# Dane-ME/keypoint-detection

Measured on AMD Instinct MI355X. Metric: images/sec @ 256x192 COCO-17 (MultiPersonKeypointModel.forward, given boxes), higher is better.
Workload: dtype fp32; 1 GPU; C2: batch 64/GPU, 256x192x3, 1 box/img, heatmap head + soft-argmax decode; model=MultiPersonKeypointModel (MobileNetV3-Small+FPN, HeatmapHead), global_batch=64, height=256, width=192, persons=1, precision=split, parallelism=dp1, streams_per_gpu=1, gather=False, gather_pipelined=False

## Files before the change

### keypoint-detection_amd/csrc/head_kernels.hip

```cpp
#include <algorithm>

#include "kpd_common.h"
#include "kpd_kernels.h"

namespace {
constexpr int HM = 56;
static_assert(HM % 4 == 0, "hm_spool / hm_sapply take 4 pixels per load instruction");
constexpr int HMP = HM * HM;
constexpr int NK = 17;
constexpr int TOPK = 64;
constexpr int FC = 128;

__device__ __forceinline__ void slotmap_image(const float* __restrict__ boxes, int b, int P, int32_t* __restrict__ slot);
__global__ __launch_bounds__(256) void topk_kernel(const float* __restrict__ stats, int tiles, int HW,
                                                   const float* __restrict__ w0, const float* __restrict__ b0,
                                                   const float* __restrict__ w2, const float* __restrict__ b2,
                                                   int32_t* __restrict__ topk, float* __restrict__ scores_out,
                                                   const float* __restrict__ boxes, int P, int32_t* __restrict__ slot,
                                                   float* __restrict__ imax, float* __restrict__ sc_zero, int sc_n) {
  extern __shared__ __attribute__((aligned(16))) float tsm[];
  float* sw0 = tsm;
  float* sw2 = sw0 + 8 * FC;
  __shared__ float avg[FC], mx[FC], h[16], sc[FC];
  const int n = blockIdx.x, tid = threadIdx.x, c = tid;
// ... 550 lines not shown
                                                       const float* __restrict__ smap, const float* __restrict__ saw,
                                                       const float* __restrict__ sab, void* __restrict__ xs,
                                                       int out_bf16, const float* __restrict__ hsc, int use_sp,
                                                       float* __restrict__ sw_out) {
  constexpr int NI = HM / 4;
  __shared__ float w[98];
  __shared__ float2 srow[7][HM + 6];
  __shared__ float ssw[HM];
  const int y = blockIdx.x, r = blockIdx.y, x = threadIdx.x, pp = x >> 4, c = x & 15;
  const float* sm = smap + (size_t)r * HMP * 2;
  const float4* src = reinterpret_cast<const float4*>(roi + ((size_t)r * HM + y) * HM * TOPK);
  float4 v[NI];
  {
#pragma unroll
    for (int i = 0; i < NI; ++i) v[i] = src[(4 * i + pp) * (TOPK / 4) + c];
    float2 sv[7];
#pragma unroll
    for (int ky = 0; ky < 7; ++ky) {
      const int iy = y + ky - 3;
      sv[ky] = (x < HM && iy >= 0 && iy < HM) ? *reinterpret_cast<const float2*>(sm + (iy * HM + x) * 2)
                                                : make_float2(0.f, 0.f);
    }
    const float w0v = saw[x], w1v = x + 64 < 98 ? saw[x + 64] : 0.f;
#pragma unroll
    for (int ky = 0; ky < 7; ++ky) {
      if (x < HM) srow[ky][x + 3] = sv[ky];
      if (x < 3) { srow[ky][x] = make_float2(0.f, 0.f); srow[ky][HM + 3 + x] = make_float2(0.f, 0.f); }
    }
    w[x] = w0v;
    if (x + 64 < 98) w[x + 64] = w1v;
  }
  __syncthreads();
  if (x < HM) {
    float a = 0.f;
#pragma unroll
    for (int ky = 0; ky < 7; ++ky) {
      const int iy = y + ky - 3;
      if (iy < 0 || iy >= HM) continue;
#pragma unroll
      for (int kx = 0; kx < 7; ++kx) {
        const int ix = x + kx - 3;
        if (ix < 0 || ix >= HM) continue;
        const float2 sv2 = srow[ky][x + kx];
        a = fmaf(w[ky * 7 + kx], sv2.x, a);
        a = fmaf(w[49 + ky * 7 + kx], sv2.y, a);
      }
    }
    ssw[x] = use_sp ? kpd_sigmoid(a + sab[0]) : 1.f;
    if (sw_out) sw_out[((size_t)r * HM + y) * HM + x] = ssw[x];
  }
  const float4 cq = reinterpret_cast<const float4*>(cw + (size_t)r * TOPK)[c];
  const float ssc = out_bf16 == 3 ? ldexpf(1.f, split_exp_of(hsc[(size_t)r * 4])) : 1.f;
  __syncthreads();
#pragma unroll
  for (int i = 0; i < NI; ++i) {
    const int px = 4 * i + pp;
    const float sw = ssw[px];
    const float4 o = make_float4((v[i].x * cq.x) * sw, (v[i].y * cq.y) * sw, (v[i].z * cq.z) * sw, (v[i].w * cq.w) * sw);
    if (out_bf16 == 3) {
      const size_t opix = hm_pos(r, y, px);
      const float ov[4] = {o.x * ssc, o.y * ssc, o.z * ssc, o.w * ssc};
      f16x4 hi, lo;
#pragma unroll
      for (int e = 0; e < 4; ++e) {
        hi[e] = (_Float16)ov[e];
        lo[e] = (_Float16)(ov[e] - (float)hi[e]);
      }
      _Float16* ob = reinterpret_cast<_Float16*>(xs) + opix * 2 * TOPK + (c >> 3) * 64 + (c & 7) * 4;
      *reinterpret_cast<f16x4*>(ob) = hi;
      *reinterpret_cast<f16x4*>(ob + 32) = lo;
    } else if (out_bf16) {
      const size_t opix = out_bf16 == 2 ? hm_pos(r, y, px)
                                        : ((size_t)r * HM + y) * HM + px;
      bf16x4 ob;
      ob[0] = (__bf16)o.x; ob[1] = (__bf16)o.y; ob[2] = (__bf16)o.z; ob[3] = (__bf16)o.w;
      *reinterpret_cast<bf16x4*>(reinterpret_cast<__bf16*>(xs) + opix * TOPK + 4 * c) = ob;
    } else {
      reinterpret_cast<float4*>(reinterpret_cast<float*>(xs) + (((size_t)r * HM + y) * HM + px) * TOPK)[c] = o;
    }
  }
}

constexpr int kAttBR = 8;
__global__ __launch_bounds__(512) void hm_attn_kernel(const float* __restrict__ roi, const float* __restrict__ cw,
                                                      const float* __restrict__ saw, const float* __restrict__ sab,
                                                      void* __restrict__ xs, int out_bf16, const float* __restrict__ hsc,
                                                      int use_sp, float* __restrict__ sw_out) {
  constexpr int NI = HM / 4, BR = kAttBR, PR = BR + 6;
  __shared__ float w[98];
  __shared__ float2 pool[PR][HM + 6];
  __shared__ float ssw[BR][HM];
  const int nb = HM / BR;
  const int nblk = gridDim.x, L = blockIdx.x;
  const int qx = nblk / 8, rx = nblk % 8, x8 = L % 8, k8 = L / 8;
  const int g = (x8 < rx ? x8 * (qx + 1) : rx * (qx + 1) + (x8 - rx) * qx) + k8;
  const int r = g / nb, y0 = (g - r * nb) * BR;
  const int tid = threadIdx.x, lane = tid & 63, wave = tid >> 6, pp = lane >> 4, c = lane & 15;
  const float4 cq = reinterpret_cast<const float4*>(cw + (size_t)r * TOPK)[c];
  if (tid < 98) w[tid] = saw[tid];
  for (int i = tid; i < PR * 6; i += 512) {
    const int rr = i / 6, cc = i - rr * 6;
    pool[rr][cc < 3 ? cc : HM + cc] = make_float2(0.f, 0.f);
  }
  for (int pr = wave; pr < PR; pr += 8) {
    const int y = y0 - 3 + pr;
    if (y < 0 || y >= HM) {
      if (lane < HM) pool[pr][lane + 3] = make_float2(0.f, 0.f);
      continue;
    }
    const float4* src = reinterpret_cast<const float4*>(roi + ((size_t)r * HM + y) * HM * TOPK);
    float4 v[NI];
#pragma unroll
    for (int i = 0; i < NI; ++i) v[i] = src[(4 * i + pp) * (TOPK / 4) + c];
#pragma unroll
    for (int i = 0; i < NI; ++i) {
      const float a = v[i].x * cq.x, b = v[i].y * cq.y, cc = v[i].z * cq.z, d = v[i].w * cq.w;
      float sm = (a + b) + (cc + d), m = fmaxf(fmaxf(a, b), fmaxf(cc, d));
      sm += dpp_f<0xB1>(sm); m = fmaxf(m, dpp_f<0xB1>(m));
      sm += dpp_f<0x4E>(sm); m = fmaxf(m, dpp_f<0x4E>(m));
      sm += dpp_f<0x124>(sm); m = fmaxf(m, dpp_f<0x124>(m));
      sm += dpp_f<0x128>(sm); m = fmaxf(m, dpp_f<0x128>(m));
      if (c == 0) pool[pr][4 * i + pp + 3] = make_float2(sm / (float)TOPK, m);
    }
  }
  __syncthreads();
  if (tid < BR * HM) {
    const int j = tid / HM, x = tid - j * HM, y = y0 + j;
    float a = 0.f;
#pragma unroll
    for (int ky = 0; ky < 7; ++ky) {
      const int iy = y + ky - 3;
      if (iy < 0 || iy >= HM) continue;
#pragma unroll
      for (int kx = 0; kx < 7; ++kx) {
        const int ix = x + kx - 3;
        if (ix < 0 || ix >= HM) continue;
        const float2 sv2 = pool[j + ky][x + kx];
        a = fmaf(w[ky * 7 + kx], sv2.x, a);
        a = fmaf(w[49 + ky * 7 + kx], sv2.y, a);
      }
    }
    ssw[j][x] = use_sp ? kpd_sigmoid(a + sab[0]) : 1.f;
    if (sw_out) sw_out[((size_t)r * HM + y) * HM + x] = ssw[j][x];
  }
  const float ssc = out_bf16 == 3 ? ldexpf(1.f, split_exp_of(hsc[(size_t)r * 4])) : 1.f;
  __syncthreads();
  {
    const int j = wave, y = y0 + j;
    const float4* src = reinterpret_cast<const float4*>(roi + ((size_t)r * HM + y) * HM * TOPK);
    float4 v[NI];
#pragma unroll
    for (int i = 0; i < NI; ++i) v[i] = src[(4 * i + pp) * (TOPK / 4) + c];
#pragma unroll
    for (int i = 0; i < NI; ++i) {
      const int px = 4 * i + pp;
      const float sw = ssw[j][px];
      const float4 o = make_float4((v[i].x * cq.x) * sw, (v[i].y * cq.y) * sw, (v[i].z * cq.z) * sw, (v[i].w * cq.w) * sw);
      if (out_bf16 == 3) {
        const size_t opix = hm_pos(r, y, px);
        const float ov[4] = {o.x * ssc, o.y * ssc, o.z * ssc, o.w * ssc};
        f16x4 hi, lo;
#pragma unroll
        for (int e = 0; e < 4; ++e) {
          hi[e] = (_Float16)ov[e];
          lo[e] = (_Float16)(ov[e] - (float)hi[e]);
        }
        _Float16* ob = reinterpret_cast<_Float16*>(xs) + opix * 2 * TOPK + (c >> 3) * 64 + (c & 7) * 4;
        *reinterpret_cast<f16x4*>(ob) = hi;
        *reinterpret_cast<f16x4*>(ob + 32) = lo;
      } else if (out_bf16) {
        const size_t opix = out_bf16 == 2 ? hm_pos(r, y, px)
                                          : ((size_t)r * HM + y) * HM + px;
        bf16x4 ob;
        ob[0] = (__bf16)o.x; ob[1] = (__bf16)o.y; ob[2] = (__bf16)o.z; ob[3] = (__bf16)o.w;
        *reinterpret_cast<bf16x4*>(reinterpret_cast<__bf16*>(xs) + opix * TOPK + 4 * c) = ob;
      } else {
        reinterpret_cast<float4*>(reinterpret_cast<float*>(xs) + (((size_t)r * HM + y) * HM + px) * TOPK)[c] = o;
      }
    }
  }
}

__global__ __launch_bounds__(64) void hm_final_kernel(const float* __restrict__ h3, const float* __restrict__ w,
                                                      const float* __restrict__ b, const int32_t* __restrict__ slot,
                                                      int P, float* __restrict__ heat_out) {
  __shared__ float sw[NK * TOPK];
  __shared__ float sb[NK];
  const int y = blockIdx.x, r = blockIdx.y, x = threadIdx.x;
  const int sl = slot[r];
  if (sl < 0) {
    if (x < HM) {
      float* dst = heat_out + ((size_t)((r / P) * P + slot_pos(sl)) * NK) * HMP + y * HM + x;
      for (int k = 0; k < NK; ++k) dst[(size_t)k * HMP] = 0.f;
    }
    return;
  }
  for (int i = x; i < NK * TOPK; i += 64) sw[i] = w[i];
  if (x < NK) sb[x] = b[x];
  __syncthreads();
  if (x >= HM) return;
  const int bimg = r / P;
  const size_t pix = ((size_t)r * HM + y) * HM + x;
  float v[TOPK];
  const float4* src = reinterpret_cast<const float4*>(h3 + pix * TOPK);
#pragma unroll
  for (int q = 0; q < TOPK / 4; ++q) {
    const float4 u = src[q];
    v[4 * q] = u.x; v[4 * q + 1] = u.y; v[4 * q + 2] = u.z; v[4 * q + 3] = u.w;
  }
  float* dst = heat_out + ((size_t)(bimg * P + sl) * NK) * HMP + y * HM + x;
  for (int k = 0; k < NK; ++k) {
    float a = 0.f;
#pragma unroll
    for (int c = 0; c < TOPK; ++c) a = fmaf(sw[k * TOPK + c], v[c], a);
    dst[(size_t)k * HMP] = kpd_sigmoid(a + sb[k]);
  }
}

__global__ __launch_bounds__(64) void decode_kernel(const float* __restrict__ heat_out,
                                                    const float* __restrict__ boxes,
                                                    const int32_t* __restrict__ slot, int P,
                                                    float* __restrict__ kpts_out, float* __restrict__ vis_out) {
  const int r = blockIdx.x, k = blockIdx.y, lane = threadIdx.x;
  const int sl = slot[r];
  const int bimg = r / P;
  if (sl < 0) {
    if (lane == 0) {
      const size_t o = (size_t)(bimg * P + slot_pos(sl)) * NK + k;
// ... 29 lines not shown
    }
    se = wave_sum(se);
    sx = wave_sum(sx);
    sy = wave_sum(sy);
    if (lane == 0) {
      const float kx = (sx / se) / (float)(HM - 1);
      const float ky = (sy / se) / (float)(HM - 1);
      const float px = fminf(fmaxf(kx * bw + (cx - bw / 2.f), 0.f), 1.f);
      const float py = fminf(fmaxf(ky * bh + (cy - bh / 2.f), 0.f), 1.f);
      kpts_out[(o + k) * 2 + 0] = px;
      kpts_out[(o + k) * 2 + 1] = py;
      const float conf = kpd_sigmoid(m);
      const int cls = (double)conf < 0.3 ? 0 : ((double)conf < 0.7 ? 1 : 2);
      vis_out[(o + k) * 3 + 0] = cls == 0 ? 1.f : 0.f;
      vis_out[(o + k) * 3 + 1] = cls == 1 ? 1.f : 0.f;
      vis_out[(o + k) * 3 + 2] = cls == 2 ? 1.f : 0.f;
    }
  }
}

}

hipError_t launch_topk(const float* stats, int N, int tiles, int HW, const float* w0, const float* b0,
                       const float* w2, const float* b2, int32_t* topk, float* scores, hipStream_t st,
                       const float* boxes, int P, int32_t* slot, float* imax, float* sc_zero, int sc_n) {
  if (slot && (!boxes || P <= 0 || P > 0xFFFF)) return hipErrorInvalidValue;
  const size_t lds = (size_t)2 * 8 * FC * 4;
  hipLaunchKernelGGL(topk_kernel, dim3(N), dim3(256), lds, st, stats, tiles, HW, w0, b0, w2, b2, topk, scores,
                     boxes, P, slot, imax, sc_zero, sc_n);
  return hipGetLastError();
}
hipError_t launch_slotmap(const float* boxes, int B, int P, int32_t* slot, hipStream_t st) {
  if (P > 0xFFFF) return hipErrorInvalidValue;
  hipLaunchKernelGGL(slotmap_kernel, dim3((B + 63) / 64), dim3(64), 0, st, boxes, B, P, slot);
  return hipGetLastError();
}
hipError_t launch_roi_align(const float* feat, int Hf, int Wf, int Cf, const int32_t* topk, const float* boxes,
                            int R, int P, float* roi, float* roi_stats, hipStream_t st, unsigned long long* stamps) {
  static const bool full_cap = kpd_diag_env("KPD_ROI_FULLCAP") != nullptr;
  if (topk) {
    static const bool direct = kpd_diag_env("KPD_ROI_DIRECT") != nullptr;
    const int cap = direct ? 0 : full_cap ? kRoiStageFloats : std::min(kRoiStageFloats, Wf * TOPK);
    hipLaunchKernelGGL((roi_align_kernel<1>), dim3(HM, R), dim3(256), cap * 4, st, feat, Hf, Wf, Cf, topk, boxes, P,
                       roi, roi_stats, cap, stamps);
  } else {
    if (Cf != 2 * TOPK) return hipErrorInvalidValue;
    static const bool direct = kpd_diag_env("KPD_ROI_DIRECT") != nullptr;
    const int cap = direct ? 0 : full_cap ? kRoiStageFloats : std::min(kRoiStageFloats, Wf * 2 * TOPK);
    hipLaunchKernelGGL((roi_align_kernel<2>), dim3(HM, R), dim3(256), cap * 4, st, feat, Hf, Wf, Cf, nullptr, boxes, P,
                       roi, nullptr, cap, stamps);
  }
  return hipGetLastError();
}
hipError_t launch_roi_kh(const float* feat, int Hf, int Wf, const int32_t* topk, const float* boxes, int R, int P,
                        float* roi, float* roi_stats, const void* w1s, int w1_exp, const float* b1, const float* w2,
                        const float* b2, const float* bound, int bdiv, int bstride, float* hsc, void* out,
                        hipStream_t st, unsigned long long* stamps) {
  if (R <= 0) return hipSuccess;
  if (!topk || !roi || !roi_stats || !w1s || !bound || bdiv < 1 || bstride < 1 || !hsc || !out)
    return hipErrorInvalidValue;
  const int cap = std::min(kRoiStageFloats, Wf * 2 * TOPK);
  const size_t lds = std::max<size_t>((size_t)cap * 4, kRoiKhLds);
  hipLaunchKernelGGL(roi_kh_kernel, dim3(HM, R), dim3(256), lds, st, feat, Hf, Wf, topk, boxes, P, roi, roi_stats,
                     cap, static_cast<const _Float16*>(w1s), w1_exp, b1, w2, b2, bound, bdiv, bstride, hsc,
                     static_cast<_Float16*>(out), stamps);
  return hipGetLastError();
}
hipError_t launch_hm_chattn(const float* roi_stats, int R, const float* w0, const float* b0, const float* w2,
                            const float* b2, float* cw, float* hsc, hipStream_t st, int abs_in) {
  hipLaunchKernelGGL(hm_chattn_kernel, dim3(R), dim3(64), 0, st, roi_stats, w0, b0, w2, b2, cw, hsc, abs_in);
  return hipGetLastError();
}
hipError_t launch_hm_spool(const float* roi, const float* cw, int R, float* smap, hipStream_t st) {
  hipLaunchKernelGGL(hm_spool_kernel, dim3(HM, R), dim3(64), 0, st, roi, cw, smap);
  return hipGetLastError();
}
hipError_t launch_hm_sapply(const float* roi, const float* cw, const float* smap, const float* saw,
                            const float* sab, int R, void* xs, int out_bf16, hipStream_t st, const float* hsc,
                            int use_sp, float* sw_out) {
  hipLaunchKernelGGL(hm_sapply_kernel, dim3(HM, R), dim3(64), 0, st, roi, cw, smap, saw, sab, xs, out_bf16, hsc,
                     use_sp, sw_out);
  return hipGetLastError();
}
hipError_t launch_hm_attn(const float* roi, const float* cw, const float* saw, const float* sab, int R, void* xs,
                          int out_bf16, hipStream_t st, const float* hsc, int use_sp, float* sw_out) {
  static_assert(HM % kAttBR == 0 && kAttBR == 8, "one wave per band row");
  if (R <= 0) return hipSuccess;
  hipLaunchKernelGGL(hm_attn_kernel, dim3((unsigned)(R * (HM / kAttBR))), dim3(512), 0, st, roi, cw, saw, sab, xs,
                     out_bf16, hsc, use_sp, sw_out);
  return hipGetLastError();
}
hipError_t launch_hm_final(const float* h3, int R, const float* w, const float* b, const int32_t* slot, int P,
                           float* heat_out, hipStream_t st) {
  hipLaunchKernelGGL(hm_final_kernel, dim3(HM, R), dim3(64), 0, st, h3, w, b, slot, P, heat_out);
  return hipGetLastError();
}
hipError_t launch_decode(const float* heat_out, const float* boxes, const int32_t* slot, int R, int P,
                         float* kpts_out, float* vis_out, hipStream_t st) {
  hipLaunchKernelGGL(decode_kernel, dim3(R, NK), dim3(64), 0, st, heat_out, boxes, slot, P, kpts_out, vis_out);
  return hipGetLastError();
}
```

### keypoint-detection_amd/csrc/kpd_kernels.h

```cpp
#pragma once
#include <hip/hip_runtime.h>
#include <stdint.h>

struct ConvArgs {
  const void* in;
  const void* wt;
  const float* bias;
  void* out;
  const float* res;
  const float* a_scale;
  float* stats;
  int N, H, W;
  int cin_p, cout_p;
  int in_cstride, out_cstride;
  int rh, rw;
  int act;
  int M;
  int tiles_per_img;
  float* amax;
  const float* post_scale;
  const float* post_shift;
  int act2, act3;
  int in_bytes, wt_bytes;
  float* splitk_ws;
// ... 130 lines not shown
struct ExDwArgs {
  const float* x;
  int Hi, Wi, cin_p;
  const float* we;
  const float* be;
  int act_e;
  const float* wd;
  const float* bd;
  int act_d, Ep;
  float* out;
  int Ho, Wo;
  float* pooled;
  int CS;
  const float* w1;
  float* part;
  int sq, C;
  unsigned long long* stamps;
  int nband;
};
size_t exdw_lds_bytes(const ExDwArgs& a, int K);
hipError_t launch_exdw(const ExDwArgs& a, int N, int K, int S, hipStream_t st);
struct SeProjArgs {
  const float* d;
  int Po, Ep;
  const float* part;
  int nsl, sq, C;
  const float *b1, *w2t, *b2;
  const float *wp, *bp;
  int cout_p, NT;
  const float* res;
  float* out;
  unsigned long long* stamps;
  const float* sesc;
};
size_t seproj_lds_bytes(const SeProjArgs& a);
hipError_t launch_seproj(const SeProjArgs& a, int N, hipStream_t st);
hipError_t launch_dwsum(const float* in, int N, int Hi, int Wi, const float* w, const float* b, int act, float* out,
                         int Ho, int Wo, int k, int s, float* part, int* ntiles, hipStream_t st);
hipError_t launch_se16_proj(const float* d, int N, int npx, int ntiles, const float* part, const float* w1,
                            const float* b1, const float* w2t, const float* b2, int sq, const float* wp,
                            const float* bp, float* out, hipStream_t st);
bool pw_small_ok(const ConvArgs& a);
hipError_t launch_pw_small(const ConvArgs& a, hipStream_t st);
hipError_t launch_se_excite(const SeProjArgs& a, int N, float* sesc, hipStream_t st);
hipError_t launch_channel_stats(const float* x, int N, int HW, int Cp, int tiles, float* stats,
                                hipStream_t st);
struct LatChainArgs {
  const float *t1, *t2, *t3, *L1, *L2, *L3;
  int c1, c2, c3, c1r, c2r, c3r, h1, w1, h2, w2, h3, w3;
  int n;
  float* lat1;
  _Float16* lat1_split;
  float* amax;
  float S1, S2, S3;
  int w_exp0, w_expE;
  const float* t0;
  _Float16* t0_split;
  int P0;
  unsigned long long* stamps;
};
size_t lateral_chain_lds_bytes(const LatChainArgs& a);
bool lateral_chain_ok(const LatChainArgs& a);
hipError_t launch_lateral_chain(const LatChainArgs& a, int N, hipStream_t st);
hipError_t launch_lateral_stream(const float* in, int cin_p, const float* w, const float* bias, const float* res,
                                 int N, int H, int W, int rh, int rw, void* out, hipStream_t st);

hipError_t launch_topk(const float* stats, int N, int tiles, int HW, const float* w0, const float* b0,
                       const float* w2, const float* b2, int32_t* topk, float* scores, hipStream_t st,
                       const float* boxes = nullptr, int P = 0, int32_t* slot = nullptr, float* imax = nullptr,
                       float* sc_zero = nullptr, int sc_n = 0);
hipError_t launch_slotmap(const float* boxes, int B, int P, int32_t* slot,
                          hipStream_t st);
hipError_t launch_roi_kh(const float* feat, int Hf, int Wf, const int32_t* topk, const float* boxes, int R, int P,
                        float* roi, float* roi_stats, const void* w1s, int w1_exp, const float* b1, const float* w2,
                        const float* b2, const float* bound, int bdiv, int bstride, float* hsc, void* out,
                        hipStream_t st, unsigned long long* stamps = nullptr);
hipError_t launch_roi_align(const float* feat, int Hf, int Wf, int Cf, const int32_t* topk,
                            const float* boxes, int R, int P, float* roi, float* roi_stats,
                            hipStream_t st, unsigned long long* stamps = nullptr);
hipError_t launch_hm_chattn(const float* roi_stats, int R, const float* w0, const float* b0,
                            const float* w2, const float* b2, float* cw, float* hsc, hipStream_t st,
                            int abs_in = 0);
hipError_t launch_hm_spool(const float* roi, const float* cw, int R, float* smap, hipStream_t st);
hipError_t launch_hm_attn(const float* roi, const float* cw, const float* saw, const float* sab, int R, void* xs,
                          int out_bf16, hipStream_t st, const float* hsc, int use_sp, float* sw_out);
hipError_t launch_hm_sapply(const float* roi, const float* cw, const float* smap, const float* saw,
                            const float* sab, int R, void* xs, int out_bf16, hipStream_t st,
                            const float* hsc = nullptr, int use_sp = 1, float* sw_out = nullptr);
hipError_t launch_hm_final(const float* h3, int R, const float* w, const float* b, const int32_t* slot,
                           int P, float* heat_out, hipStream_t st);
hipError_t launch_decode(const float* heat_out, const float* boxes, const int32_t* slot, int R, int P,
                         float* kpts_out, float* vis_out, hipStream_t st);

hipError_t launch_nms(const float* boxes, const float* scores, int n, float thr, int max_out,
                      int32_t* keep, int32_t* n_keep, void* scratch, size_t scratch_bytes, hipStream_t st);
hipError_t launch_nms_sets(const float* boxes, const float* scores, int sets, int n, float thr, int max_out,
                           int max_keep, int32_t* keep, int32_t* n_keep, void* scratch, hipStream_t st, int filter,
                           float* out_boxes, float* out_scores);
size_t nms_scratch_bytes(int n);

hipError_t launch_adaptive_pool56(const float* in, int B, int Hf, int Wf, int C, float* out, hipStream_t st);
bool person_detect_fits(int Wf);
hipError_t launch_person_detect(const float* feat, int B, int Hf, int Wf, const float* w, const float* bias,
                                const float* anchors, int img_h, int img_w, float conf, float* cand_boxes,
                                float* cand_scores, hipStream_t st);
hipError_t launch_person_decode(const float* head, int B, int hc, const float* anchors, int img_h, int img_w,
                                float conf, float* cand_boxes, float* cand_scores, hipStream_t st);
hipError_t launch_kh_att(float* x, const float* sa1, const float* w, const float* b, size_t npix, hipStream_t st);
hipError_t launch_kh_att2(const float* x, const void* w1s, int w1_exp, const float* b1, const float* w2,
                          const float* b2, int R, const float* bound, int bdiv, int bstride, float* hsc, void* out,
                          hipStream_t st);
hipError_t launch_kh_att_split(const float* x, const float* sa1, const float* w, const float* b, int R,
                               const float* bound, int bdiv, int bstride, float* hsc, void* out, hipStream_t st);
hipError_t launch_kh_pool(const float* in, int R, int C, int o, float* out, int out_stride, hipStream_t st);
hipError_t launch_kh_final(const float* lin_r, int r_stride, const float* lin_v, int v_stride, const float* ln_rg,
                           const float* ln_rb, const float* w_r, const float* b_r, const float* ln_vg,
                           const float* ln_vb, const float* w_v, const float* b_v, const int32_t* slot, int R, int P,
                           float* kh_kpts, float* kh_vis, hipStream_t st);

int kpd_fail_einval(const char* msg);
int kpd_fail_hip(hipError_t e, const char* where);

hipError_t launch_decode_planes(const float* heat, int planes, int H, int W, int mode, float param, float* kpts,
                                float* scores, float* vis, hipStream_t st);
hipError_t launch_roi_align_nchw(const float* feat, int C, int H, int W, const float* rois, int R, int oh, int ow,
                                 float scale, int sr, int aligned, float* out, hipStream_t st);
hipError_t launch_nchw_rows_to_nhwc(const float* in, int N, int C, int H, int W, float* out, float* stats,
                                    hipStream_t st, float* amax = nullptr, int amax_stride = 0);
hipError_t launch_nhwc_to_nchw(const float* in, int N, int HW, int C, float* out, hipStream_t st);
hipError_t launch_nhwc_pad_to_nchw(const float* in, int N, int HW, int C, int Cp, float* out, hipStream_t st);
hipError_t launch_nchw_to_nhwc_pad(const float* in, int N, int HW, int C, int Cp, float* out, hipStream_t st);
hipError_t launch_nchw_channel_stats(const float* x, int N, int C, int HW, float* stats, hipStream_t st);
hipError_t launch_gather_planes(const float* x, int N, int C, int HW, const int32_t* idx, int K, float* out,
                                hipStream_t st);
hipError_t launch_conv1x1_nchw(const float* x, int N, int Cin, int HW, const float* w, const float* b, int Cout,
                               float* out, hipStream_t st);
hipError_t launch_fill(float* p, long n, float v, hipStream_t st);

hipError_t launch_conv3_forward(const float* x, const float* w, const float* b, int N, int C, int H, int W, int O,
                                float* y, hipStream_t st);
size_t conv3_wgrad_slices(int N, int H, int W);
hipError_t launch_conv3_backward(const float* x, const float* w, const float* gy, int N, int C, int H, int W, int O,
                                 float* gx, float* gw, float* gb, float* wgrad_part, hipStream_t st);
```

### keypoint-detection_amd/csrc/kpd_plan.hip

```cpp
#include <cmath>
#include <cstdlib>
#include <cstdio>
#include <cstring>
#include <initializer_list>
#include <map>
#include <memory>
#include <string>
#include <vector>

#include "../../include/kpd.h"
#include "kpd_common.h"
#include "kpd_kernels.h"

namespace {

thread_local std::string g_err;

int fail(int code, const std::string& msg) {
  g_err = msg;
  return code;
}

#define HIP_TRY(expr)                                                                          \
  do {                                                                                         \
// ... 995 lines not shown
      chk(pack_bn_affine(p, B + "bn1", rb[i]->cout_p ? rb[i]->cout_p : 64, bs[i], bt[i], missing));
    }
    chk(pack_conv(p, R + "2.weight", R + "2.bias", R + "3", 1e-5, 3, false, p->kh_c3, missing));
    chk(pack_conv(p, R + "7.weight", R + "7.bias", "", 0, 1, false, p->kh_lr, missing));
    chk(pack_plain(p, R + "8.weight", &p->kh_lnr_g, missing, 256));
    chk(pack_plain(p, R + "8.bias", &p->kh_lnr_b, missing, 256));
    chk(pack_plain(p, R + "11.weight", &p->kh_fr_w, missing, 34 * 256));
    chk(pack_plain(p, R + "11.bias", &p->kh_fr_b, missing, 34));
    chk(pack_conv(p, V + "0.weight", V + "0.bias", V + "1", 1e-5, 3, false, p->kh_v1, missing));
    chk(pack_conv(p, V + "5.weight", V + "5.bias", "", 0, 1, false, p->kh_lv, missing));
    chk(pack_plain(p, V + "6.weight", &p->kh_lnv_g, missing, 128));
    chk(pack_plain(p, V + "6.bias", &p->kh_lnv_b, missing, 128));
    chk(pack_plain(p, V + "9.weight", &p->kh_fv_w, missing, 51 * 128));
    chk(pack_plain(p, V + "9.bias", &p->kh_fv_b, missing, 51));
    if (rc == KPD_OK && missing.empty()) {
      const int in = p->kh_lr.cin;
      int o = 1;
      while (16 * (o + 1) * (o + 1) <= in) ++o;
      if (16 * o * o != in || p->kh_c3.cout != 16 || p->kh_v1.cout != 32 || p->kh_lv.cin != 512 ||
          p->kh_sa1.cin != 128 || p->kh_sa1.cout != 64)
        return fail(KPD_EINVAL, "KEYPOINT_HEAD shape not supported (needs in 128, regression 32, square pool)");
      p->kh_o = o;
    }
    const bool std_kh = p->kh_rb1.cin == 128 && p->kh_rb1.cout == 64 && p->kh_ds1.w && p->kh_rb2.cin == 64 &&
                        p->kh_rb2.cout == 32 && p->kh_ds2.w && p->kh_c3.cin == 32 && p->kh_v1.cin == 128;
    static const bool no_kh_split = kpd_diag_env("KPD_NO_KH_SPLIT") != nullptr;
    if (precision != KPD_PRECISION_FP32 && rc == KPD_OK && missing.empty() && std_kh && !no_kh_split) {
      chk(pack_split_kh(p, p->kh_s[0], 128, 128, 10, {{&p->kh_rb1, &p->kh_ds1, p->kh_bn1a_s, p->kh_bn1a_t, 0},
                                                      {&p->kh_v1, nullptr, nullptr, nullptr, 64}}));
      p->kh_s[0].ns = 64; p->kh_s[0].nf = 32;
      chk(pack_split_kh(p, p->kh_s[1], 64, 64, 10, {{&p->kh_rb2, &p->kh_ds2, p->kh_bn1b_s, p->kh_bn1b_t, 0}}));
      p->kh_s[1].ns = 32; p->kh_s[1].nf = 0;
      chk(pack_split_kh(p, p->kh_s[2], 32, 64, 9, {{&p->kh_c3, nullptr, nullptr, nullptr, 0}}));
      p->kh_s[2].ns = 0; p->kh_s[2].nf = 16;
      if (p->kh_sa1.cin_p == 128 && p->kh_sa1.cout_p == 64) chk(pack_split_1x1(p, p->kh_sa1));
      p->kh_split = rc == KPD_OK;
    }
  }
  if (!missing.empty()) return fail(KPD_ESTATE, "missing tensors: " + missing);
  if (rc != KPD_OK) return rc;
  if (p->has_fpn && (p->fpn0.cin != 128 || p->fpn0.cout != 128)) return fail(KPD_EINVAL, "fpn_convs.0 must be 128->128");
  if (p->has_hm && (p->hm1.cin != 64 || p->hm3.cout != 64 || p->hm1.cout != p->hm2.cin || p->hm2.cout != p->hm3.cin))
    return fail(KPD_EINVAL, "heatmap head channel chain mismatch");
  if (p->has_body && p->bn[0].cfg.cin != 16) return fail(KPD_EINVAL, "bad body");
  p->finalized = true;
  ++p->ws_epoch;
  return KPD_OK;
}

static int max_pass_images(int H, int W) {
  const long hf = (H - 1) / 2 + 1, wf = (W - 1) / 2 + 1;
  const long by_extent = 0x7fffffffL / (hf * wf * 512);
  return (int)std::max(1L, std::min<long>(kFpn0xMaxImg, by_extent));
}

static bool fpn0x_ok(const kpd_plan* p, const Dims& d) {
  static const bool no_lin = kpd_diag_env("KPD_NO_FPN0X") != nullptr;
  return p->precision != KPD_PRECISION_FP32 && !no_lin && p->fpn0x.w0 != nullptr && d.Hf == 4 * d.h[3] &&
         d.Wf == 4 * d.w[3] && (long)((d.h[3] * d.w[3] + 255) / 256) * 256 < 65536;
}

static int ensure_work(kpd_plan* p, const Dims& d, int k, hipStream_t st) {
  if (p->have_work[k] && d.fits(p->dims[k])) return KPD_OK;
  if (p->have_work[k]) HIP_TRY(hipDeviceSynchronize());
  Work w;
  const size_t need = carve(p, d, nullptr, w);
  if (need > p->ws_bytes[k]) {
    if (p->ws[k]) HIP_TRY(hipFree(p->ws[k]));
    p->ws[k] = nullptr;
    HIP_TRY(hipMalloc(&p->ws[k], need));
    p->ws_bytes[k] = need;
  }
  carve(p, d, reinterpret_cast<char*>(p->ws[k]), p->work[k]);
  p->work[k].sc_dirty = true;
  ++p->ws_epoch;
  if (hm_padded(p)) HIP_TRY(hipMemsetAsync(p->ws[k], 0, need, st));
  p->dims[k] = d;
  p->have_work[k] = true;
  return KPD_OK;
}

static int run_heatmap_head(kpd_plan* p, Work& w, int R, int P, float* heat_out, hipStream_t st, int parts,
                            float* sw_out, unsigned long long* stamps2, unsigned long long* stamps3,
                            unsigned long long* stamps1 = nullptr, int abs_in = 0) {
  std::unique_ptr<Stage> att_stage(new Stage(p, "hm_attention", st));
  const bool hsplit = p->precision == KPD_PRECISION_SPLIT;
  HIP_TRY(launch_hm_chattn(w.roi_stats, R, p->hca_w0, p->hca_b0, p->hca_w2, p->hca_b2, w.cw,
                           hsplit ? w.hsc : nullptr, st, abs_in));
  if (!(parts & KPD_HEAD_CHANNEL_ATT)) HIP_TRY(launch_fill(w.cw, (long)R * 64, 1.f, st));
  const bool bf = p->precision == KPD_PRECISION_MIXED;
  const int xs_mode = hsplit ? 3 : bf ? (hm_padded(p) ? 2 : 1) : 0;
  static const bool att_2k = kpd_diag_env("KPD_HM_ATT_2K") != nullptr;
  if (att_2k) {
    HIP_TRY(launch_hm_spool(w.roi, w.cw, R, w.smap, st));
    HIP_TRY(launch_hm_sapply(w.roi, w.cw, w.smap, p->sa_w, p->sa_b, R, w.xs, xs_mode, st, w.hsc,
                             (parts & KPD_HEAD_SPATIAL_ATT) != 0, sw_out));
  } else {
    HIP_TRY(launch_hm_attn(w.roi, w.cw, p->sa_w, p->sa_b, R, w.xs, xs_mode, st, w.hsc,
                           (parts & KPD_HEAD_SPATIAL_ATT) != 0, sw_out));
  }
  att_stage.reset();
  if (!(parts & KPD_HEAD_CONVS)) return KPD_OK;
  const HmSplit sp1{w.hsc, 0.f, 1.f, 0, p->hm1.bc, p->hm1.bs, 0, 1};
  const HmSplit sp2{w.hsc, p->hm1.bc, p->hm1.bs, 0, p->hm2.bc, p->hm2.bs, 1, -1};
  const HmSplit sp3{w.hsc, p->hm2.bc, p->hm2.bs, 1, 0.f, 0.f, -1, -1};
  std::unique_ptr<Stage> c1(new Stage(p, "hm_conv1", st));
  if (int rc = hm_conv(p, p->hm1, w.xs, R, 64, w.h1, 1, st, nullptr, stamps1, &sp1)) return rc;
  c1.reset();
  std::unique_ptr<Stage> c2(new Stage(p, "hm_conv2", st));
  if (int rc = hm_conv(p, p->hm2, w.h1, R, p->hm1.cout_p, w.h2, 1, st, nullptr, stamps2, &sp2))
    return rc;
  c2.reset();
  std::unique_ptr<Stage> c3(new Stage(p, "hm_conv3", st));
  static const bool no_fin_fuse = kpd_diag_env("KPD_NO_FINAL_FUSE") != nullptr;
  const bool fin_fused = (p->hm3.bf16 || p->hm3.ws) && p->hm3.cout_p == 64 && (!no_fin_fuse || p->hm3.ws);
  const HmFinal fin{p->fin_w, p->fin_b, w.slot, P, heat_out};
  if (int rc = hm_conv(p, p->hm3, w.h2, R, p->hm2.cout_p, w.h3, 2, st, fin_fused ? &fin : nullptr, stamps3, &sp3))
    return rc;
  c3.reset();
  if (!fin_fused) HIP_TRY(launch_hm_final(w.h3, R, p->fin_w, p->fin_b, w.slot, P, heat_out, st));
  return KPD_OK;
}

static int run_keypoint_head(kpd_plan* p, Work& w, int R, int P, float* kh_kpts, float* kh_vis, hipStream_t st,
                             const float* bound, int bdiv, int bstride, bool x_ready = false,
                             unsigned long long* const* stamps = nullptr) {
  const size_t px = (size_t)R * 3136;
  if (p->kh_split && w.kxs) {
    static const bool att1 = kpd_diag_env("KPD_KH_ATT1") != nullptr;
    if (x_ready) {
    } else if (att1 || !p->kh_sa1.ws) {
      if (int rc = conv(p->kh_sa1, w.kx, R, 56, 56, 128, w.ksa, ACT_RELU6, nullptr, 0, 0, nullptr, nullptr, 0, 0, st))
        return rc;
      HIP_TRY(launch_kh_att_split(w.kx, w.ksa, p->kh_sa2_w, p->kh_sa2_b, R, bound, bdiv, bstride, w.hsc, w.kxs, st));
    } else {
      HIP_TRY(launch_kh_att2(w.kx, p->kh_sa1.ws, p->kh_sa1.w_exp, p->kh_sa1.b, p->kh_sa2_w, p->kh_sa2_b, R, bound,
                             bdiv, bstride, w.hsc, w.kxs, st));
    }
    const void* ins[3] = {w.kxs, w.kr1s, w.kr2s};
    void* outs[3] = {w.kr1s, w.kr2s, nullptr};
    float* outf[3] = {w.kv1, nullptr, w.kr3};
    for (int i = 0; i < 3; ++i) {
      const KhSplit& k = p->kh_s[i];
      HmConvArgs h{};
      h.in = ins[i]; h.wt = k.ws; h.bias = k.b; h.out = outs[i]; h.outf = outf[i];
      h.R = R; h.cin = k.cin; h.cout = k.cout; h.ntap = k.ntap; h.ns = k.ns; h.nf = k.nf;
      h.kh_ps = k.ps; h.kh_pt = k.pt; h.kh_bd = k.ntap == 10 ? k.bd : nullptr;
      h.split = 1; h.hsc = w.hsc; h.w_exp = k.w_exp;
      h.in_c = i == 0 ? 0.f : 6.f; h.in_s = i == 0 ? 1.f : 0.f; h.in_idx = 2;
      h.out_c = 6.f; h.out_s = 0.f; h.out_idx = k.ns > 0 ? 2 : -1; h.amax_idx = -1;
      h.stamps = stamps ? stamps[i] : nullptr;
      HIP_TRY(launch_hmconv(h, st));
    }
    const int o = p->kh_o, kr = pad16(16 * o * o);
    if (kr != 16 * o * o) HIP_TRY(hipMemsetAsync(w.kpr, 0, sizeof(float) * R * kr, st));
    HIP_TRY(launch_kh_pool(w.kr3, R, 16, o, w.kpr, kr, st));
    HIP_TRY(launch_kh_pool(w.kv1, R, 32, 4, w.kpv, 512, st));
    if (int rc = conv(p->kh_lr, w.kpr, R, 1, 1, kr, w.klr, ACT_NONE, nullptr, 0, 0, nullptr, nullptr, 0, 0, st))
      return rc;
    if (int rc = conv(p->kh_lv, w.kpv, R, 1, 1, 512, w.klv, ACT_NONE, nullptr, 0, 0, nullptr, nullptr, 0, 0, st))
      return rc;
    HIP_TRY(launch_kh_final(w.klr, p->kh_lr.cout_p, w.klv, p->kh_lv.cout_p, p->kh_lnr_g, p->kh_lnr_b, p->kh_fr_w,
                            p->kh_fr_b, p->kh_lnv_g, p->kh_lnv_b, p->kh_fv_w, p->kh_fv_b, w.slot, R, P, kh_kpts,
                            kh_vis, st));
    return KPD_OK;
  }
  if (int rc = conv(p->kh_sa1, w.kx, R, 56, 56, 128, w.ksa, ACT_RELU6, nullptr, 0, 0, nullptr, nullptr, 0, 0, st))
    return rc;
  HIP_TRY(launch_kh_att(w.kx, w.ksa, p->kh_sa2_w, p->kh_sa2_b, px, st));
  const float* id1 = w.kx;
  if (p->kh_ds1.w) {
    if (int rc = conv(p->kh_ds1, w.kx, R, 56, 56, 128, w.kds1, ACT_NONE, nullptr, 0, 0, nullptr, nullptr, 0, 0, st))
      return rc;
    id1 = w.kds1;
  }
  if (int rc = conv_post(p->kh_rb1, w.kx, R, 56, 56, 128, w.krb1, ACT_RELU6, p->kh_bn1a_s, p->kh_bn1a_t,
                         ACT_RELU6, id1, ACT_RELU6, st))
    return rc;
  const float* id2 = w.krb1;
  if (p->kh_ds2.w) {
    if (int rc = conv(p->kh_ds2, w.krb1, R, 56, 56, p->kh_rb1.cout_p, w.kds2, ACT_NONE, nullptr, 0, 0, nullptr,
                      nullptr, 0, 0, st))
// ... 565 lines not shown
  p->graph_abandon_next = enable == 2;
  return KPD_OK;
}

int kpd_plan_set_detector(kpd_plan* p, float conf_threshold, float nms_iou_threshold) {
  if (!p) return fail(KPD_EINVAL, "null plan");
  if (!(conf_threshold >= 0.f && conf_threshold <= 1.f) || !(nms_iou_threshold >= 0.f && nms_iou_threshold <= 1.f))
    return fail(KPD_EINVAL, "thresholds must be in [0, 1]");
  p->det_conf = conf_threshold;
  p->det_iou = nms_iou_threshold;
  ++p->ws_epoch;
  return KPD_OK;
}

int kpd_plan_timing(kpd_plan* p, int enable) {
  if (!p) return fail(KPD_EINVAL, "null plan");
  p->timing = enable != 0;
  if (p->timing)
    for (auto& kv : p->timers) kv.second.used = 0;
  return KPD_OK;
}

int kpd_plan_timing_stage(kpd_plan* p, const char* stage) {
  if (!p) return fail(KPD_EINVAL, "null plan");
  p->timing_only = stage ? stage : "";
  return KPD_OK;
}

int kpd_plan_timing_query(kpd_plan* p, const char* stage, double* total_ms, int* count) {
  if (!p || !stage || !total_ms || !count) return fail(KPD_EINVAL, "null argument");
  *total_ms = 0.0;
  *count = 0;
  auto it = p->timers.find(stage);
  if (it == p->timers.end()) return KPD_OK;
  for (size_t i = 0; i < it->second.used; ++i) {
    auto& e = it->second.ev[i];
    HIP_TRY(hipEventSynchronize(e.second));
    float ms = 0.f;
    HIP_TRY(hipEventElapsedTime(&ms, e.first, e.second));
    *total_ms += ms;
  }
  *count = (int)it->second.used;
  return KPD_OK;
}

int kpd_debug_copy(kpd_plan* p, const char* name, void* dst, size_t bytes, size_t* size_out, void* stream) {
  if (!p || !name) return fail(KPD_EINVAL, "null argument");
  auto it = p->debug.find(name);
  if (it == p->debug.end()) return fail(KPD_EINVAL, std::string("no debug buffer ") + name);
  if (size_out) *size_out = it->second.second;
  if (!dst) return KPD_OK;
  if (bytes < it->second.second) return fail(KPD_EINVAL, "destination too small");
  HIP_TRY(hipMemcpyAsync(dst, it->second.first, it->second.second, hipMemcpyDeviceToDevice,
                         reinterpret_cast<hipStream_t>(stream)));
  return KPD_OK;
}


static int op_work(kpd_plan* p, int R, int flags, hipStream_t st, Work** w) {
  Dims d;
  d.B = 0; d.NB = R; d.P = 1; d.flags = flags | (p->has_kh ? KPD_FLAG_DUAL_HEAD : 0);
  if (int rc = ensure_work(p, d, kpd_plan::kOpWs, st)) return rc;
  *w = &p->work[kpd_plan::kOpWs];
  g_splitk = (*w)->splitk;
  return KPD_OK;
}

int kpd_heatmap_head(kpd_plan* p, const float* x, int R, int H, int W, int parts, float* heat, float* ch_w,
                     float* sp_w, void* stream) {
  if (!p || !p->finalized) return fail(KPD_ESTATE, "plan not finalized");
  if (!p->has_hm) return fail(KPD_ESTATE, "plan has no heatmap_head weights");
  if (R < 0 || H != 56 || W != 56) return fail(KPD_EINVAL, "HeatmapHead input must be [R][64][56][56]");
  if (parts & ~KPD_HEAD_ALL) return fail(KPD_EINVAL, "unknown HeatmapHead parts");
  if (R == 0) return KPD_OK;
  if (!x || ((parts & KPD_HEAD_CONVS) && !heat)) return fail(KPD_EINVAL, "null pointer");
  hipStream_t st = reinterpret_cast<hipStream_t>(stream);
  HIP_TRY(hipSetDevice(p->device));
  Work* w = nullptr;
  if (int rc = op_work(p, R, 0, st, &w)) return rc;
  const bool hsplit = p->precision == KPD_PRECISION_SPLIT;
  if (hsplit) HIP_TRY(hipMemsetAsync(w->hsc, 0, sizeof(float) * 4 * R, st));
  HIP_TRY(launch_nchw_rows_to_nhwc(x, R, 64, 56, 56, w->roi, w->roi_stats, st, hsplit ? w->hsc + 2 : nullptr, 4));
  HIP_TRY(hipMemsetAsync(w->slot, 0, sizeof(int32_t) * R, st));
  if (int rc = run_heatmap_head(p, *w, R, 1, heat, st, parts, sp_w, nullptr, nullptr, nullptr, 1)) return rc;
  if (ch_w) HIP_TRY(hipMemcpyAsync(ch_w, w->cw, sizeof(float) * R * 64, hipMemcpyDeviceToDevice, st));
  return KPD_OK;
}

int kpd_keypoint_head(kpd_plan* p, const float* x, int R, int H, int W, float* kpts, float* vis, void* stream) {
  if (!p || !p->finalized) return fail(KPD_ESTATE, "plan not finalized");
  if (!p->has_kh) return fail(KPD_ESTATE, "plan has no keypoint_head weights");
  if (R < 0 || H != 56 || W != 56) return fail(KPD_EINVAL, "KEYPOINT_HEAD input must be [R][128][56][56]");
  if (R == 0) return KPD_OK;
  if (!x || !kpts || !vis) return fail(KPD_EINVAL, "null pointer");
  hipStream_t st = reinterpret_cast<hipStream_t>(stream);
  HIP_TRY(hipSetDevice(p->device));
  Work* w = nullptr;
  if (int rc = op_work(p, R, KPD_FLAG_DUAL_HEAD, st, &w)) return rc;
  if (p->kh_split) HIP_TRY(hipMemsetAsync(w->hsc, 0, sizeof(float) * 4 * R, st));
  HIP_TRY(launch_nchw_rows_to_nhwc(x, R, 128, 56, 56, w->kx, nullptr, st, p->kh_split ? w->hsc + 2 : nullptr, 4));
  HIP_TRY(hipMemsetAsync(w->slot, 0, sizeof(int32_t) * R, st));
  return run_keypoint_head(p, *w, R, 1, kpts, vis, st, w->hsc + 2, 1, 4);
}

int kpd_backbone(kpd_plan* p, const float* image, int B, int C, int H, int W, float* out0, float* out1, float* out2,
                 float* out3, void* stream) {
  if (!p || !p->finalized) return fail(KPD_ESTATE, "plan not finalized");
  if (!p->has_body || !p->has_fpn) return fail(KPD_ESTATE, "plan lacks backbone.body / backbone.fpn weights");
  for (int i = 0; i < 3; ++i)
    if (!p->fpn_lv[i].w) return fail(KPD_ESTATE, "plan lacks backbone.fpn.fpn_convs.1-3 weights");
  if (!image || B <= 0 || H < 32 || W < 32) return fail(KPD_EINVAL, "bad image shape");
  if (C != p->in_ch) return fail(KPD_EINVAL, "image channels do not match backbone in_channels");
  float* outs[4] = {out0, out1, out2, out3};
  for (float* o : outs)
    if (!o) return fail(KPD_EINVAL, "null output pointer");
  hipStream_t st = reinterpret_cast<hipStream_t>(stream);
  HIP_TRY(hipSetDevice(p->device));
  int h[12], wd[12];
  h[0] = (H - 1) / 2 + 1; wd[0] = (W - 1) / 2 + 1;
  for (int i = 0; i < 11; ++i) {
    const int k = kBneck[i].k, s = kBneck[i].s, pd = (k - 1) / 2;
    h[i + 1] = (h[i] + 2 * pd - k) / s + 1;
    wd[i + 1] = (wd[i] + 2 * pd - k) / s + 1;
  }
  const int lh[4] = {h[0], h[3], h[8], h[11]}, lw[4] = {wd[0], wd[3], wd[8], wd[11]};
  const int cap = max_pass_images(H, W), npass = (B + cap - 1) / cap;
  for (int q = 0; q < npass; ++q) {
    const int b0 = (int)((long)B * q / npass), b1 = (int)((long)B * (q + 1) / npass), nb = b1 - b0;
    p->keep_laterals = true;
    const int rc1 = forward_one(p, 0, false, image + (size_t)b0 * C * H * W, nb, C, H, W, nullptr, 0, 0, 0, nullptr,
                                nullptr, nullptr, nullptr, nullptr, nullptr, nullptr, st);
    p->keep_laterals = false;
    if (rc1) return rc1;
    Work& w = p->work[0];
    HIP_TRY(launch_nhwc_to_nchw(w.feat, nb, lh[0] * lw[0], 128, outs[0] + (size_t)b0 * 128 * lh[0] * lw[0], st));
    for (int i = 1; i < 4; ++i) {
      if (int rc = conv(p->fpn_lv[i - 1], w.lat[i], nb, lh[i], lw[i], 128, w.feat, ACT_RELU, nullptr, 0, 0, nullptr,
                        nullptr, 0, 0, st))
        return rc;
      HIP_TRY(launch_nhwc_to_nchw(w.feat, nb, lh[i] * lw[i], 128, outs[i] + (size_t)b0 * 128 * lh[i] * lw[i], st));
    }
  }
  return KPD_OK;
}

int kpd_backbone_body(kpd_plan* p, const float* image, int B, int C, int H, int W, float* feat0, float* feat1,
                      float* feat2, float* feat3, void* stream) {
  if (!p || !p->finalized) return fail(KPD_ESTATE, "plan not finalized");
  if (!p->has_body) return fail(KPD_ESTATE, "plan lacks backbone.body weights");
  if (!image || B <= 0 || H < 32 || W < 32) return fail(KPD_EINVAL, "bad image shape");
  if (C != p->in_ch) return fail(KPD_EINVAL, "image channels do not match backbone in_channels");
  float* outs[4] = {feat0, feat1, feat2, feat3};
  for (float* o : outs)
    if (!o) return fail(KPD_EINVAL, "null output pointer");
  hipStream_t st = reinterpret_cast<hipStream_t>(stream);
  HIP_TRY(hipSetDevice(p->device));
  int h[12], wd[12];
  h[0] = (H - 1) / 2 + 1; wd[0] = (W - 1) / 2 + 1;
  for (int i = 0; i < 11; ++i) {
    const int k = kBneck[i].k, s = kBneck[i].s, pd = (k - 1) / 2;
    h[i + 1] = (h[i] + 2 * pd - k) / s + 1;
    wd[i + 1] = (wd[i] + 2 * pd - k) / s + 1;
  }
  const int lv[4] = {0, 3, 8, 11};
  const int cap = max_pass_images(H, W), npass = (B + cap - 1) / cap;
  for (int q = 0; q < npass; ++q) {
    const int b0 = (int)((long)B * q / npass), b1 = (int)((long)B * (q + 1) / npass), nb = b1 - b0;
// ... 171 lines not shown
```

Baseline: 40710 images/s.

## Fuse channel-attention MLP into the fused heatmap attention kernel

The separate channel-attention kernel (and optional fill) is folded into hm_attn_kernel. Each block now recomputes the avg/max pooled stats, the small two-layer MLP and the split scale u0 from roi_stats. The first band block writes hsc and optionally cw, while two waves do the MLP and the other six prefetch roi rows. This removes a kernel launch and a dependency round-trip per forward, at the cost of redundant MLP work across the 7 blocks per ROI and more shared-memory and register pressure in the 512-thread kernel.

```diff
diff --git a/keypoint-detection_amd/csrc/head_kernels.hip b/keypoint-detection_amd/csrc/head_kernels.hip
--- a/keypoint-detection_amd/csrc/head_kernels.hip
+++ b/keypoint-detection_amd/csrc/head_kernels.hip
@@ -656,36 +656,125 @@
 }
 
 constexpr int kAttBR = 8;
-__global__ __launch_bounds__(512) void hm_attn_kernel(const float* __restrict__ roi, const float* __restrict__ cw,
+__global__ __launch_bounds__(512) void hm_attn_kernel(const float* __restrict__ roi,
+                                                      const float* __restrict__ roi_stats,
+                                                      const float* __restrict__ cw0, const float* __restrict__ cb0,
+                                                      const float* __restrict__ cw2, const float* __restrict__ cb2,
+                                                      int chan_att, int abs_in, float* __restrict__ cw_out,
                                                       const float* __restrict__ saw, const float* __restrict__ sab,
-                                                      void* __restrict__ xs, int out_bf16, const float* __restrict__ hsc,
+                                                      void* __restrict__ xs, int out_bf16, float* __restrict__ hsc,
                                                       int use_sp, float* __restrict__ sw_out) {
-  constexpr int NI = HM / 4, BR = kAttBR, PR = BR + 6;
+  constexpr int NI = HM / 4, BR = kAttBR, PR = BR + 6, W0S = TOPK + 4;
+  static_assert(PR == 14, "pooled rows: 6 + 8 over the waves");
   __shared__ float w[98];
   __shared__ float2 pool[PR][HM + 6];
   __shared__ float ssw[BR][HM];
+  __shared__ __attribute__((aligned(16))) float sav[2][TOPK], sw0[4 * W0S], sw2[4 * TOPK], sb2[TOPK];
+  __shared__ float sb0[4], su0;
   const int nb = HM / BR;
   const int nblk = gridDim.x, L = blockIdx.x;
   const int qx = nblk / 8, rx = nblk % 8, x8 = L % 8, k8 = L / 8;
   const int g = (x8 < rx ? x8 * (qx + 1) : rx * (qx + 1) + (x8 - rx) * qx) + k8;
   const int r = g / nb, y0 = (g - r * nb) * BR;
   const int tid = threadIdx.x, lane = tid & 63, wave = tid >> 6, pp = lane >> 4, c = lane & 15;
-  const float4 cq = reinterpret_cast<const float4*>(cw + (size_t)r * TOPK)[c];
-  if (tid < 98) w[tid] = saw[tid];
+  float4 v[NI];
+  if (wave < 2) {
+    float vr[HM];
+    const float* st = roi_stats + (size_t)r * HM * 2 * TOPK + wave * TOPK + lane;
+#pragma unroll
+    for (int row = 0; row < HM; ++row) vr[row] = st[row * 2 * TOPK];
+    const float w0a = cw0[tid], w0b = cw0[tid + 2 * TOPK], w2a = cw2[tid], w2b = cw2[tid + 2 * TOPK];
+    const float b2v = cb2[lane], b0v = cb0[lane & 3], sawv = saw[min(tid, 97)];
+    if (wave == 0) {
+      float s = 0.f;
+#pragma unroll
+      for (int row = 0; row < HM; ++row) s += vr[row];
+      sav[0][lane] = s / (float)HMP;
+    } else {
+      const float absv = hsc && abs_in ? hsc[(size_t)r * 4 + 2] : 0.f;
+      float m = -INFINITY;
+#pragma unroll
+      for (int row = 0; row < HM; ++row) m = fmaxf(m, vr[row]);
+      sav[1][lane] = m;
+      if (hsc) {
+        float u0 = fmaxf(wave_max(m), 0.f);
+        if (abs_in) u0 = fmaxf(u0, absv);
+        if (lane == 0) {
+          su0 = u0;
+          if (y0 == 0) {
+            hsc[(size_t)r * 4] = u0;
+            hsc[(size_t)r * 4 + 1] = 0.f;
+          }
+        }
+      }
+    }
+    sw0[wave * W0S + lane] = w0a;
+    sw0[(wave + 2) * W0S + lane] = w0b;
+    sw2[tid] = w2a;
+    sw2[tid + 2 * TOPK] = w2b;
+    if (wave == 0) sb2[lane] = b2v;
+    if (tid < 4) sb0[tid] = b0v;
+    if (tid < 98) w[tid] = sawv;
+  } else {
+    const int yf = min(max(y0 - 3 + wave - 2, 0), HM - 1);
+    const float4* src = reinterpret_cast<const float4*>(roi + ((size_t)r * HM + yf) * HM * TOPK);
+#pragma unroll
+    for (int i = 0; i < NI; ++i) v[i] = src[(4 * i + pp) * (TOPK / 4) + c];
+  }
   for (int i = tid; i < PR * 6; i += 512) {
     const int rr = i / 6, cc = i - rr * 6;
     pool[rr][cc < 3 ? cc : HM + cc] = make_float2(0.f, 0.f);
   }
-  for (int pr = wave; pr < PR; pr += 8) {
-    const int y = y0 - 3 + pr;
+  __syncthreads();
+  float4 cq;
+  {
+    const float4* wr = reinterpret_cast<const float4*>(sw0 + (lane & 3) * W0S);
+    const float4* vq = reinterpret_cast<const float4*>(sav[(lane >> 2) & 1]);
+    float a = sb0[lane & 3];
+#pragma unroll
+    for (int k4 = 0; k4 < TOPK / 4; ++k4) {
+      const float4 wk = wr[k4], xk = vq[k4];
+      a = fmaf(wk.x, xk.x, a);
+      a = fmaf(wk.y, xk.y, a);
+      a = fmaf(wk.z, xk.z, a);
+      a = fmaf(wk.w, xk.w, a);
+    }
+    const float h = fmaxf(a, 0.f);
+    float ha[4], hx[4];
+#pragma unroll
+    for (int j = 0; j < 4; ++j) {
+      ha[j] = __builtin_bit_cast(float, __builtin_amdgcn_readlane(__builtin_bit_cast(int, h), j));
+      hx[j] = __builtin_bit_cast(float, __builtin_amdgcn_readlane(__builtin_bit_cast(int, h), 4 + j));
+    }
+    const float4 bq = reinterpret_cast<const float4*>(sb2)[c];
+    const float bb[4] = {bq.x, bq.y, bq.z, bq.w};
+    float o[4];
+#pragma unroll
+    for (int e = 0; e < 4; ++e) {
+      const float4 wq = reinterpret_cast<const float4*>(sw2)[4 * c + e];
+      const float wj[4] = {wq.x, wq.y, wq.z, wq.w};
+      float oa = bb[e], om = bb[e];
+#pragma unroll
+      for (int j = 0; j < 4; ++j) {
+        oa = fmaf(wj[j], ha[j], oa);
+        om = fmaf(wj[j], hx[j], om);
+      }
+      o[e] = chan_att ? kpd_sigmoid(oa + om) : 1.f;
+    }
+    cq = make_float4(o[0], o[1], o[2], o[3]);
+    if (cw_out && y0 == 0 && tid < TOPK / 4) reinterpret_cast<float4*>(cw_out + (size_t)r * TOPK)[c] = cq;
+  }
+  for (int pass = wave < 2 ? 1 : 0; pass < 2; ++pass) {
+    const int pr = pass ? 6 + wave : wave - 2, y = y0 - 3 + pr;
     if (y < 0 || y >= HM) {
       if (lane < HM) pool[pr][lane + 3] = make_float2(0.f, 0.f);
       continue;
     }
-    const float4* src = reinterpret_cast<const float4*>(roi + ((size_t)r * HM + y) * HM * TOPK);
-    float4 v[NI];
-#pragma unroll
-    for (int i = 0; i < NI; ++i) v[i] = src[(4 * i + pp) * (TOPK / 4) + c];
+    if (pass) {
+      const float4* src = reinterpret_cast<const float4*>(roi + ((size_t)r * HM + y) * HM * TOPK);
+#pragma unroll
+      for (int i = 0; i < NI; ++i) v[i] = src[(4 * i + pp) * (TOPK / 4) + c];
+    }
 #pragma unroll
     for (int i = 0; i < NI; ++i) {
       const float a = v[i].x * cq.x, b = v[i].y * cq.y, cc = v[i].z * cq.z, d = v[i].w * cq.w;
@@ -717,7 +806,7 @@
     ssw[j][x] = use_sp ? kpd_sigmoid(a + sab[0]) : 1.f;
     if (sw_out) sw_out[((size_t)r * HM + y) * HM + x] = ssw[j][x];
   }
-  const float ssc = out_bf16 == 3 ? ldexpf(1.f, split_exp_of(hsc[(size_t)r * 4])) : 1.f;
+  const float ssc = out_bf16 == 3 ? ldexpf(1.f, split_exp_of(su0)) : 1.f;
   __syncthreads();
   {
     const int j = wave, y = y0 + j;
@@ -913,12 +1002,15 @@
                      use_sp, sw_out);
   return hipGetLastError();
 }
-hipError_t launch_hm_attn(const float* roi, const float* cw, const float* saw, const float* sab, int R, void* xs,
-                          int out_bf16, hipStream_t st, const float* hsc, int use_sp, float* sw_out) {
+hipError_t launch_hm_attn(const float* roi, const float* roi_stats, const float* w0, const float* b0,
+                          const float* w2, const float* b2, int chan_att, int abs_in, float* cw_out,
+                          const float* saw, const float* sab, int R, void* xs, int out_bf16, hipStream_t st,
+                          float* hsc, int use_sp, float* sw_out) {
   static_assert(HM % kAttBR == 0 && kAttBR == 8, "one wave per band row");
   if (R <= 0) return hipSuccess;
-  hipLaunchKernelGGL(hm_attn_kernel, dim3((unsigned)(R * (HM / kAttBR))), dim3(512), 0, st, roi, cw, saw, sab, xs,
-                     out_bf16, hsc, use_sp, sw_out);
+  if (out_bf16 == 3 && !hsc) return hipErrorInvalidValue;
+  hipLaunchKernelGGL(hm_attn_kernel, dim3((unsigned)(R * (HM / kAttBR))), dim3(512), 0, st, roi, roi_stats, w0, b0,
+                     w2, b2, chan_att, abs_in, cw_out, saw, sab, xs, out_bf16, hsc, use_sp, sw_out);
   return hipGetLastError();
 }
 hipError_t launch_hm_final(const float* h3, int R, const float* w, const float* b, const int32_t* slot, int P,
diff --git a/keypoint-detection_amd/csrc/kpd_kernels.h b/keypoint-detection_amd/csrc/kpd_kernels.h
--- a/keypoint-detection_amd/csrc/kpd_kernels.h
+++ b/keypoint-detection_amd/csrc/kpd_kernels.h
@@ -236,8 +236,10 @@
                             const float* w2, const float* b2, float* cw, float* hsc, hipStream_t st,
                             int abs_in = 0);
 hipError_t launch_hm_spool(const float* roi, const float* cw, int R, float* smap, hipStream_t st);
-hipError_t launch_hm_attn(const float* roi, const float* cw, const float* saw, const float* sab, int R, void* xs,
-                          int out_bf16, hipStream_t st, const float* hsc, int use_sp, float* sw_out);
+hipError_t launch_hm_attn(const float* roi, const float* roi_stats, const float* w0, const float* b0,
+                          const float* w2, const float* b2, int chan_att, int abs_in, float* cw_out,
+                          const float* saw, const float* sab, int R, void* xs, int out_bf16, hipStream_t st,
+                          float* hsc, int use_sp, float* sw_out);
 hipError_t launch_hm_sapply(const float* roi, const float* cw, const float* smap, const float* saw,
                             const float* sab, int R, void* xs, int out_bf16, hipStream_t st,
                             const float* hsc = nullptr, int use_sp = 1, float* sw_out = nullptr);
diff --git a/keypoint-detection_amd/csrc/kpd_plan.hip b/keypoint-detection_amd/csrc/kpd_plan.hip
--- a/keypoint-detection_amd/csrc/kpd_plan.hip
+++ b/keypoint-detection_amd/csrc/kpd_plan.hip
@@ -1101,22 +1101,24 @@
 
 static int run_heatmap_head(kpd_plan* p, Work& w, int R, int P, float* heat_out, hipStream_t st, int parts,
                             float* sw_out, unsigned long long* stamps2, unsigned long long* stamps3,
-                            unsigned long long* stamps1 = nullptr, int abs_in = 0) {
+                            unsigned long long* stamps1 = nullptr, int abs_in = 0, bool keep_cw = false) {
   std::unique_ptr<Stage> att_stage(new Stage(p, "hm_attention", st));
   const bool hsplit = p->precision == KPD_PRECISION_SPLIT;
-  HIP_TRY(launch_hm_chattn(w.roi_stats, R, p->hca_w0, p->hca_b0, p->hca_w2, p->hca_b2, w.cw,
-                           hsplit ? w.hsc : nullptr, st, abs_in));
-  if (!(parts & KPD_HEAD_CHANNEL_ATT)) HIP_TRY(launch_fill(w.cw, (long)R * 64, 1.f, st));
   const bool bf = p->precision == KPD_PRECISION_MIXED;
   const int xs_mode = hsplit ? 3 : bf ? (hm_padded(p) ? 2 : 1) : 0;
   static const bool att_2k = kpd_diag_env("KPD_HM_ATT_2K") != nullptr;
   if (att_2k) {
+    HIP_TRY(launch_hm_chattn(w.roi_stats, R, p->hca_w0, p->hca_b0, p->hca_w2, p->hca_b2, w.cw,
+                             hsplit ? w.hsc : nullptr, st, abs_in));
+    if (!(parts & KPD_HEAD_CHANNEL_ATT)) HIP_TRY(launch_fill(w.cw, (long)R * 64, 1.f, st));
     HIP_TRY(launch_hm_spool(w.roi, w.cw, R, w.smap, st));
     HIP_TRY(launch_hm_sapply(w.roi, w.cw, w.smap, p->sa_w, p->sa_b, R, w.xs, xs_mode, st, w.hsc,
                              (parts & KPD_HEAD_SPATIAL_ATT) != 0, sw_out));
   } else {
-    HIP_TRY(launch_hm_attn(w.roi, w.cw, p->sa_w, p->sa_b, R, w.xs, xs_mode, st, w.hsc,
-                           (parts & KPD_HEAD_SPATIAL_ATT) != 0, sw_out));
+    HIP_TRY(launch_hm_attn(w.roi, w.roi_stats, p->hca_w0, p->hca_b0, p->hca_w2, p->hca_b2,
+                           (parts & KPD_HEAD_CHANNEL_ATT) != 0, abs_in, keep_cw ? w.cw : nullptr, p->sa_w, p->sa_b,
+                           R, w.xs, xs_mode, st, hsplit ? w.hsc : nullptr, (parts & KPD_HEAD_SPATIAL_ATT) != 0,
+                           sw_out));
   }
   att_stage.reset();
   if (!(parts & KPD_HEAD_CONVS)) return KPD_OK;
@@ -1848,7 +1850,8 @@
   if (hsplit) HIP_TRY(hipMemsetAsync(w->hsc, 0, sizeof(float) * 4 * R, st));
   HIP_TRY(launch_nchw_rows_to_nhwc(x, R, 64, 56, 56, w->roi, w->roi_stats, st, hsplit ? w->hsc + 2 : nullptr, 4));
   HIP_TRY(hipMemsetAsync(w->slot, 0, sizeof(int32_t) * R, st));
-  if (int rc = run_heatmap_head(p, *w, R, 1, heat, st, parts, sp_w, nullptr, nullptr, nullptr, 1)) return rc;
+  if (int rc = run_heatmap_head(p, *w, R, 1, heat, st, parts, sp_w, nullptr, nullptr, nullptr, 1, ch_w != nullptr))
+    return rc;
   if (ch_w) HIP_TRY(hipMemcpyAsync(ch_w, w->cw, sizeof(float) * R * 64, hipMemcpyDeviceToDevice, st));
   return KPD_OK;
 }
```

After: 40770 images/s, median of 3. Within noise of the previous version (+0.1%).
